# zyddnys/manga-image-translator

Hardware: AMD Instinct MI355X
Metric: pages/sec end-to-end (detect+OCR+inpaint), 2048x1456 (higher is better)
Workload: dtype f32

## Files before the change

manga_image_translator_amd/csrc/conv_gemm.hip:

```cpp
#include "conv_gemm_table.h"
#include <atomic>

using namespace mitcg;

#define G(name, fam, BM, BN, BK, ...) \
    extern template void mitcg::launch_##fam##_group<BM, BN, BK, __VA_ARGS__>(const mitcg::GroupArgs &, int, int, hipStream_t);
#include "conv_gemm_group_cfgs.inc"
#undef G

namespace {

int64_t max_a_offset(const MitConvGemm &p) {
    if (p.a_bs < 0 || p.a_ys < 0 || p.a_xs < 0) return -1;
    int tmax = 0;
    for (int t = 0; t < p.ntaps; ++t) {
        if (p.tap_off[t] < 0) return -1;
        if (p.tap_off[t] > tmax) tmax = p.tap_off[t];
    }
    return (int64_t)(p.NB - 1) * p.a_bs + (int64_t)(p.Hi - 1) * p.a_ys + (int64_t)(p.Wi - 1) * p.a_xs + p.Cin + tmax;
}
bool fast_eligible(const MitConvGemm &p, int BK) {
    if (p.Cin % BK || p.ntaps > FAST_MAX_TAPS) return false;
    const int64_t maxoff = max_a_offset(p);
    return maxoff >= 0 && maxoff < 0x7fffffffLL;
}

bool split_eligible(const MitConvGemm &p, int BK) {
    if (!p.w_split || (reinterpret_cast<uintptr_t>(p.w_split) & 15) || (p.ws_zs0 & 7)) return false;
    if (p.w_zs1 != 0 || (p.Kw & 7) || p.ntaps * p.Cin > p.Kw) return false;
    if ((int64_t)3 * (p.Kw >> 3) * p.ldw > 0x7fffffffLL) return false;
    return fast_eligible(p, BK);
}

bool buf_eligible(const MitConvGemm &p) {
    const int64_t maxoff = max_a_offset(p);
    return maxoff >= 0 && maxoff * 4 < 0x80000000LL && (int64_t)3 * (p.Kw >> 3) * p.ldw * 16 < 0x80000000LL;
}
int buf_form(const MitConvGemm &p, int c) { return buf_eligible(p) ? kCfgs[c].twin : c; }

bool gemv_eligible(const MitConvGemm &p, int lpr) {
    if (p.N > 4 || p.Z != 1 || p.Cin % (4 * lpr) || (int64_t)p.NB * p.Ho > 65535) return false;
    if ((int64_t)p.ntaps * p.Cin * (p.N == 1 ? 1 : 4) * 4 > 60 * 1024) return false;
    if (p.c.nsplit || p.pre.nsplit || p.post.nsplit || p.lut_rows) return false;
    return true;
}

std::atomic<int> g_gemm_mode{-1};
int gemm_mode_now() {
    int m = g_gemm_mode.load(std::memory_order_relaxed);
    if (m < 0) {
        const char *v = getenv("MIT_GEMM_SPLIT");
        m = (v && *v) ? atoi(v) : 6;
        if (m != 6 && m != 9) m = 0;
        g_gemm_mode.store(m, std::memory_order_relaxed);
    }
    return m;
}

std::atomic<long long> g_split_min{0};
int64_t split_min_now() { return g_split_min.load(std::memory_order_relaxed); }

struct TileSet {
    int n32;
    int narrow, wide;
    int small;
    int64_t small_max;
    int small_k32;
};
constexpr TileSet kGenericTiles = {CFG("128x32x16"), CFG("128x64x16"), CFG("128x128x16"), -1, 0, -1};
constexpr TileSet kFp32Tiles = {CFG("fast128x32x16w4c"), CFG("fast128x64x16w5c"), CFG("fast128x128x16w4c"), CFG("fast64x64x16w8c"), 1280, -1};
constexpr TileSet kP6Tiles = {CFG("split128x32x16p6o"), CFG("split128x64x16p6o"), CFG("split128x128x16p6o"), CFG("split64x64x16p6o"), 768, CFG("split64x64x32p6o")};
constexpr TileSet kP9Tiles = {CFG("split128x32x16p9m"), CFG("split128x64x16p9"), CFG("split128x128x16p9m"), CFG("split64x64x16p9m"), 768, CFG("split64x64x32p9m")};
constexpr TileSet kP1Tiles = {-1, CFG("split128x64x32p1o"), CFG("split128x128x32p1o"), CFG("split64x64x32p1o"), 768, -1};

int64_t tiles128(const MitConvGemm &p, int64_t M) { return ((M + 127) / 128) * ((p.N + 63) / 64); }

int ladder(const TileSet &s, const MitConvGemm &p, int64_t M, int exact = -1) {
    if (p.N <= 32 && s.n32 >= 0) return s.n32;
    const int rem = p.N % 128;
    int c = (p.N <= 64 || (rem != 0 && rem <= 64)) ? s.narrow : s.wide;
    if (exact >= 0) c = exact;
    if (s.small >= 0 && p.Z == 1 && tiles128(p, M) < s.small_max) {
        c = s.small;
        if (s.small_k32 >= 0 && ((M + 63) / 64) * ((p.N + 63) / 64) <= 512 && split_eligible(p, 32)) c = s.small_k32;
    }
    return c;
}

int exact_n_p6(const MitConvGemm &p) {
    if (p.Z != 1) return -1;
    const int K = p.ntaps * p.Cin;
    if ((p.N == 160 || p.N == 320) && K >= 512) return CFG("split128x160x16p6o");
    if (p.N > 64 && p.N <= 96 && K >= 256) return CFG("split128x96x16p6o");
    if (p.N == 192 && K >= 256) return CFG("split128x192x16p6o");
    return -1;
}

int pick_cfg(const MitConvGemm &p, int64_t M) {
    if (p.nprod == 1) {
        if (!split_eligible(p, 32)) return buf_form(p, CFG("split64x64x16p1o"));
        return buf_form(p, ladder(kP1Tiles, p, M, p.N % 192 == 0 ? CFG("split128x192x32p1o") : -1));
    }
    if (gemv_eligible(p, 16)) return p.N == 1 ? CFG("gemv16n1") : CFG("gemv16");
    if (gemv_eligible(p, 4)) return p.N == 1 ? CFG("gemv4n1") : CFG("gemv4");
    const int mode = gemm_mode_now();
    if ((mode == 6 || mode == 9) && p.w_split && split_eligible(p, 16) && tiles128(p, M) * p.Z >= split_min_now())
        return buf_form(p, mode == 6 ? ladder(kP6Tiles, p, M, exact_n_p6(p)) : ladder(kP9Tiles, p, M));
    if (!fast_eligible(p, 16)) return ladder(kGenericTiles, p, M);
    if (p.N > 32 && M > 128 && M <= 192 && p.Z >= 8) return CFG("fast192x64x16w4c");
    return ladder(kFp32Tiles, p, M);
}

struct ProbeRec {
    hipEvent_t start, stop;
    int cfg;
    double exec_flops, alg_flops;
    int M, N, K, ntaps, Z, act;
    double wino_bytes;
};
std::mutex g_probe_mu;
bool g_probe_on = false;
std::vector<ProbeRec> g_probe;
thread_local double g_next_alg_flops = -1.0;

}

extern "C" int mit_prof_enable(int on) {
    std::lock_guard<std::mutex> lk(g_probe_mu);
    for (auto &r : g_probe) {
        (void)hipEventDestroy(r.start);
        (void)hipEventDestroy(r.stop);
    }
    g_probe.clear();
    g_probe_on = on != 0;
    mit_probe_reset(on != 0);
    return 0;
}

extern "C" int mit_prof_tag_next(double alg_flops) {
    g_next_alg_flops = alg_flops;
    return 0;
}

extern "C" int mit_prof_dump(const char *path) {
    if (!path) return mit_set_error("mit_prof_dump: null path");
    std::lock_guard<std::mutex> lk(g_probe_mu);
    FILE *f = fopen(path, "w");
    if (!f) return mit_set_error("mit_prof_dump: cannot open %s", path);
    fprintf(f, "tile,M,N,K,taps,Z,act,ms,exec_flops,alg_flops,wino_bytes\n");
    for (auto &r : g_probe) {
        float ms = 0.f;
        if (hipEventSynchronize(r.stop) != hipSuccess || hipEventElapsedTime(&ms, r.start, r.stop) != hipSuccess) {
            fclose(f);
            return mit_set_error("mit_prof_dump: event query failed");
        }
        fprintf(f, "%s,%d,%d,%d,%d,%d,%d,%.6f,%.0f,%.0f,%.0f\n", kCfgs[r.cfg].name, r.M, r.N, r.K, r.ntaps, r.Z, r.act, ms, r.exec_flops,
                r.alg_flops, r.wino_bytes);
    }
    fclose(f);
    return 0;
}

extern "C" int mit_prof_read(MitProfStat *stats, int max_cfgs, int *n_cfgs) {
    if (!stats || !n_cfgs) return mit_set_error("mit_prof_read: null");
    std::lock_guard<std::mutex> lk(g_probe_mu);
    const int n = max_cfgs < kNumCfgs ? max_cfgs : kNumCfgs;
    for (int i = 0; i < n; ++i) {
        stats[i].launches = 0;
        stats[i].ms = stats[i].exec_flops = stats[i].alg_flops = 0.0;
    }
    for (auto &r : g_probe) {
        MIT_CHECK_HIP(hipEventSynchronize(r.stop));
        float ms = 0.f;
        MIT_CHECK_HIP(hipEventElapsedTime(&ms, r.start, r.stop));
        if (r.cfg < n) {
            stats[r.cfg].launches += 1;
            stats[r.cfg].ms += ms;
            stats[r.cfg].exec_flops += r.exec_flops;
            stats[r.cfg].alg_flops += r.alg_flops;
        }
    }
    *n_cfgs = n;
    return 0;
}

extern "C" const char *mit_conv_gemm_config_name(int cfg) {
    if (cfg < 0 || cfg >= kNumCfgs) return nullptr;
    return kCfgs[cfg].name;
}

extern "C" const char *mit_conv_gemm_config_kernel(int cfg) {
    if (cfg < 0 || cfg >= kNumCfgs) return nullptr;
    return kCfgs[cfg].kernel;
}

namespace {
bool map_vec_ok(const MitTensorMap &m, bool split_ok = false) {
    if (m.nsplit != 0 && !(split_ok && !(m.nsplit & 3) && !(m.nhi & 3))) return false;
    return !(reinterpret_cast<uintptr_t>(m.base) & 15) && !((m.zs1 | m.zs0 | m.bs | m.ys | m.xs) & 3);
}
bool vec_epilogue_ok(const MitConvGemm &p) {
    if ((p.N & 3) || !map_vec_ok(p.c, true)) return false;
    if (p.pre.base && !map_vec_ok(p.pre)) return false;
    if (p.post.base && !map_vec_ok(p.post)) return false;
    if (p.lut_rows && ((p.lut_ld & 3) || (reinterpret_cast<uintptr_t>(p.lut1) & 15) || (reinterpret_cast<uintptr_t>(p.lut2) & 15))) return false;
    return !(reinterpret_cast<uintptr_t>(p.scale) & 15) && !(reinterpret_cast<uintptr_t>(p.bias) & 15);
}

int64_t list_rows(const MitConvGemm &p) { return (int64_t)p.NB * ((p.Ho + 7) / 8) * ((p.Wo + 7) / 8) * 64; }
int64_t rows_of(const MitConvGemm &p) { return p.live_blocks ? list_rows(p) : (int64_t)p.NB * p.Ho * p.Wo; }

int validate(const MitConvGemm *d, MitConvGemm &p) {
    if (!d) return mit_set_error("mit_conv_gemm: null descriptor");
    p = *d;
    if (p.act & MIT_ACT_VEC_OK) return mit_set_error("mit_conv_gemm: reserved activation bits set");
    if (vec_epilogue_ok(p)) p.act |= MIT_ACT_VEC_OK;
    if (!p.a || !p.w || !p.c.base) return mit_set_error("mit_conv_gemm: null operand");
    if (p.Cin <= 0 || (p.Cin & 3)) return mit_set_error("mit_conv_gemm: Cin must be a positive multiple of 4 (got %d)", p.Cin);
    if ((p.ldw & 3) || (p.Nw & 3)) return mit_set_error("mit_conv_gemm: ldw/Nw must be multiples of 4 (ldw=%lld Nw=%d)", (long long)p.ldw, p.Nw);
    if (p.ntaps <= 0 || p.ntaps > MIT_MAX_TAPS) return mit_set_error("mit_conv_gemm: ntaps %d out of range", p.ntaps);
    if (p.NB <= 0 || p.Ho <= 0 || p.Wo <= 0 || p.N <= 0 || p.Z <= 0 || p.zdiv <= 0)
        return mit_set_error("mit_conv_gemm: empty problem");
    if ((reinterpret_cast<uintptr_t>(p.a) & 15) || (reinterpret_cast<uintptr_t>(p.w) & 15))
        return mit_set_error("mit_conv_gemm: operands must be 16-byte aligned");
    if ((p.a_xs & 3) || (p.a_ys & 3) || (p.a_bs & 3) || (p.a_zs0 & 3) || (p.a_zs1 & 3) || (p.w_zs0 & 3) || (p.w_zs1 & 3))
        return mit_set_error("mit_conv_gemm: strides must be multiples of 4 elements");
    for (int t = 0; t < p.ntaps; ++t)
        if (p.tap_off[t] & 3) return mit_set_error("mit_conv_gemm: tap_off must be multiples of 4");
    if (p.pad_mode == MIT_PAD_REFLECT) {
        for (int t = 0; t < p.ntaps; ++t) {
            int ady = p.tap_dy[t] < 0 ? -p.tap_dy[t] : p.tap_dy[t];
            int adx = p.tap_dx[t] < 0 ? -p.tap_dx[t] : p.tap_dx[t];
            if (ady >= p.Hi || adx >= p.Wi) return mit_set_error("mit_conv_gemm: reflect pad larger than input");
        }
    }
    if ((int64_t)p.NB * p.Ho * p.Wo > 0x7fffffffLL) return mit_set_error("mit_conv_gemm: M too large");
    if (p.lut_rows) {
        if (!p.lut1 || !p.lut2 || p.lut_ld < p.N) return mit_set_error("mit_conv_gemm: lut_rows needs lut1, lut2 and lut_ld >= N");
        if (p.Z != 1) return mit_set_error("mit_conv_gemm: the row-lookup epilogue is for Z == 1 launches");
        if (p.lut_ld > 0x7fff) return mit_set_error("mit_conv_gemm: lut_ld too large (row offsets are 16-bit row x lut_ld in 32 bits)");
    }
    if (p.live_blocks || p.live_start) {
        if (!p.live_blocks || !p.live_start) return mit_set_error("mit_conv_gemm: a live-block list needs live_blocks and live_start");
        if ((reinterpret_cast<uintptr_t>(p.live_blocks) | reinterpret_cast<uintptr_t>(p.live_start)) & 3) return mit_set_error("mit_conv_gemm: live_blocks / live_start must be 4-byte aligned");
        if (p.Z != 1) return mit_set_error("mit_conv_gemm: a live-block list is for Z == 1 launches");
        if (p.lut_rows) return mit_set_error("mit_conv_gemm: a live-block list together with lut_rows is not implemented");
        if (p.live_img0 < 0) return mit_set_error("mit_conv_gemm: live_img0 must be >= 0 (got %d)", p.live_img0);
        if (list_rows(p) > 0x7fffffffLL) return mit_set_error("mit_conv_gemm: M too large");
    } else if (p.live_img0 != 0) {
        return mit_set_error("mit_conv_gemm: live_img0 without a live-block list");
    }
    if (p.wino_m) {
        if (!p.live_blocks) return mit_set_error("mit_conv_gemm: wino_m needs the 8 x 8 block row order (live_blocks / live_start; list every block for a dense layer)");
        if (p.ntaps != 1 || p.sy != 1 || p.sx != 1) return mit_set_error("mit_conv_gemm: wino_m is for one tap with stride 1 (got %d taps, stride %d x %d)", p.ntaps, p.sy, p.sx);
        if (p.pre.base) return mit_set_error("mit_conv_gemm: wino_m together with a pre operand is not implemented");
        if (p.c.nsplit || (p.post.base && p.post.nsplit)) return mit_set_error("mit_conv_gemm: wino_m with a column-split map is not implemented");
        if ((p.N & 3) || p.wino_n != p.N) return mit_set_error("mit_conv_gemm: wino_m needs N %% 4 == 0 and wino_n == N (N=%d wino_n=%d)", p.N, p.wino_n);
        if (p.wino_th != (p.Ho + 3) / 4 || p.wino_tw != (p.Wo + 3) / 4)
            return mit_set_error("mit_conv_gemm: wino_th x wino_tw must be ceil(Ho / 4) x ceil(Wo / 4) (got %d x %d for %d x %d)", p.wino_th, p.wino_tw, p.Ho, p.Wo);
        if (p.wino_zs < (int64_t)p.NB * p.wino_th * p.wino_tw * p.wino_n) return mit_set_error("mit_conv_gemm: wino_zs is shorter than one slice of tiles (NB * wino_th * wino_tw * wino_n)");
        if (reinterpret_cast<uintptr_t>(p.wino_m) & 3) return mit_set_error("mit_conv_gemm: wino_m must be 4-byte aligned");
    }
    if (p.Z > 65535) return mit_set_error("mit_conv_gemm: Z too large");
    if (p.nprod != 0 && p.nprod != 1) return mit_set_error("mit_conv_gemm: nprod must be 0 (the GEMM mode) or 1 (one bf16 product) (got %d)", p.nprod);
    if (p.nprod == 1 && !p.w_split) return mit_set_error("mit_conv_gemm: nprod = 1 needs w_split (mit_gemm_split_pack): there is no fp32 fallback for a requested precision");
    return 0;
}

int images_per_run(const MitConvGemm &p) {
    if (p.Z != 1 || p.NB <= 1) return p.NB;
    MitConvGemm q = p;
    q.NB = 1;
    const bool want_buf = (gemm_mode_now() == 6 || p.nprod == 1) && p.w_split != nullptr && split_eligible(p, 16) && buf_eligible(q);
    auto run_ok = [&](const MitConvGemm &r) { return fast_eligible(r, 16) && (!want_buf || buf_eligible(r)); };
    if (p.Cin % 16 != 0 || p.ntaps > FAST_MAX_TAPS || p.a_bs <= 0 || run_ok(p) || !fast_eligible(q, 16)) return p.NB;
    int nb = p.NB;
    while (nb > 1) {
        q.NB = nb;
        if (run_ok(q)) break;
        nb = (nb + 1) / 2;
    }
    return nb;
}
MitConvGemm run_of(const MitConvGemm &p, int b0, int nb) {
    MitConvGemm r = p;
    r.NB = nb;
    r.a += (int64_t)b0 * p.a_bs;
    r.c.base += (int64_t)b0 * p.c.bs;
    if (p.pre.base) r.pre.base += (int64_t)b0 * p.pre.bs;
    if (p.post.base) r.post.base += (int64_t)b0 * p.post.bs;
    if (p.lut_rows) r.lut_rows += (int64_t)b0 * p.Ho * p.Wo;
    if (p.wino_m) r.wino_m += (int64_t)b0 * p.wino_th * p.wino_tw * p.wino_n;
    if (p.live_blocks) r.live_start += b0, r.live_img0 += b0;
    return r;
}

int plan_run(const MitConvGemm &p, int cfg, int *tile) {
    const int64_t M = rows_of(p);
    if (p.nprod == 1) {
        if (!split_eligible(p, 16))
            return mit_set_error("mit_conv_gemm: nprod = 1 needs the split tiles' preconditions (Cin %% 16 == 0, <= %d taps, 32-bit element offsets, 16-byte aligned w_split with w_zs1 == 0 and Kw %% 8 == 0): there is no fp32 fallback for a requested precision", FAST_MAX_TAPS);
        if (cfg >= 0 && cfg < kNumCfgs && kCfgs[cfg].nprod() != 1) return mit_set_error("mit_conv_gemm: nprod = 1 with tile %s, which is not a one-product tile", kCfgs[cfg].name);
    }
    if (cfg < 0) cfg = pick_cfg(p, M);
    if (cfg >= kNumCfgs) return mit_set_error("mit_conv_gemm: bad cfg %d", cfg);
    const CfgEntry &c = kCfgs[cfg];
    const bool fast = c.family == TileFamily::fast, split = c.family == TileFamily::split, gemv = c.family == TileFamily::gemv;
    if (p.lut_rows) {
        if (!fast && !split)
            return mit_set_error("mit_conv_gemm: the row-lookup epilogue (lut_rows) needs a fast or split tile (Cin %% 16 == 0, <= %d taps); this launch takes %s", FAST_MAX_TAPS, c.name);
        if (!(p.act & MIT_ACT_VEC_OK)) return mit_set_error("mit_conv_gemm: lut_rows needs the float4 epilogue (N %% 4 == 0, 16-byte aligned maps, tables and lut_ld %% 4 == 0)");
        if (p.post.base) return mit_set_error("mit_conv_gemm: lut_rows together with a post residual is not implemented");
        if ((p.act & 0xff) != MIT_ACT_NONE && (p.act & 0xff) != MIT_ACT_RELU) return mit_set_error("mit_conv_gemm: lut_rows is implemented for act none / relu");
    }
    if (p.live_blocks && !fast && !split)
        return mit_set_error("mit_conv_gemm: a live-block list needs a fast or split tile (Cin %% 16 == 0, <= %d taps, N > 4); this launch takes %s", FAST_MAX_TAPS, c.name);
    if (gemv && (!gemv_eligible(p, c.lanes_per_row()) || p.N > c.BN))
        return mit_set_error("mit_conv_gemm: cfg %s needs N <= %d, Z == 1, unsplit maps and Cin %% %d == 0", c.name, c.BN, 4 * c.lanes_per_row());
    if (split && !split_eligible(p, c.BK))
        return mit_set_error("mit_conv_gemm: cfg %s needs w_split (mit_gemm_split_pack, 16-byte aligned, w_zs1 == 0, Kw %% 8 == 0) and the fast tiles' preconditions", c.name);
    if (fast && !fast_eligible(p, c.BK))
        return mit_set_error("mit_conv_gemm: cfg %s needs Cin %% %d == 0, <= %d taps and 32-bit element offsets", c.name, c.BK, FAST_MAX_TAPS);
    if ((M + c.BM - 1) / c.BM * ((p.N + c.BN - 1) / c.BN) > 0x7fffffffLL) return mit_set_error("mit_conv_gemm: grid too large");
    *tile = cfg;
    return 0;
}

int launch_run(const MitConvGemm &p, int cfg, hipStream_t hs) {
    const CfgEntry &c = kCfgs[cfg];
    const int M = (int)rows_of(p);
    const int MT = (M + c.BM - 1) / c.BM;
    const int NT = (p.N + c.BN - 1) / c.BN;
    const int Ktot = p.ntaps * p.Cin;
    const int KT = (Ktot + c.BK - 1) / c.BK;
    const double tagged = g_next_alg_flops;
    g_next_alg_flops = -1.0;
    if (g_probe_on) {
        std::lock_guard<std::mutex> lk(g_probe_mu);
        ProbeRec r;
        MIT_CHECK_HIP(hipEventCreate(&r.start));
// ... 235 lines not shown
```

manga_image_translator_amd/csrc/conv_gemm_cfgs.inc:

```
X(0, "128x128x16", generic, 128, 128, 16, 2, 2)
X(0, "128x64x16", generic, 128, 64, 16, 2, 2)
X(0, "128x32x16", generic, 128, 32, 16, 4, 1)
X(1, "fast128x128x16w4c", fast, 128, 128, 16, 1, 4, 4, 4)
X(1, "fast128x64x16w5c", fast, 128, 64, 16, 2, 2, 5, 4)
X(1, "fast192x64x16w4c", fast, 192, 64, 16, 2, 2, 4, 4)
X(1, "fast64x64x16w8c", fast, 64, 64, 16, 2, 2, 8, 4)
X(1, "fast128x32x16w4c", fast, 128, 32, 16, 4, 1, 4, 4)
X(0, "gemv16", gemv, 8, 4, 4, 16)
X(0, "gemv4", gemv, 8, 4, 4, 4)
X(0, "gemv16n1", gemv, 8, 1, 4, 16)
X(0, "gemv4n1", gemv, 4, 1, 4, 4)
X(4, "split128x128x16p6o", split, 128, 128, 16, 2, 2, 3, 6, 385)
X(4, "split128x128x16p9m", split, 128, 128, 16, 2, 2, 3, 9, 129)
X(4, "split128x64x16p6o", split, 128, 64, 16, 2, 2, 3, 6, 385)
X(3, "split128x64x16p9", split, 128, 64, 16, 2, 2, 2, 9, 0)
X(3, "split64x64x16p6o", split, 64, 64, 16, 2, 2, 4, 6, 385)
X(3, "split64x64x16p9m", split, 64, 64, 16, 2, 2, 4, 9, 129)
X(3, "split64x64x32p6o", split, 64, 64, 32, 2, 2, 3, 6, 385)
X(3, "split64x64x32p9m", split, 64, 64, 32, 2, 2, 3, 9, 129)
X(3, "split128x32x16p6o", split, 128, 32, 16, 4, 1, 4, 6, 385)
X(3, "split128x32x16p9m", split, 128, 32, 16, 4, 1, 4, 9, 129)
X(3, "split128x160x16p6o", split, 128, 160, 16, 4, 1, 2, 6, 385)
X(3, "split128x96x16p6o", split, 128, 96, 16, 4, 1, 3, 6, 385)
X(3, "split128x192x16p6o", split, 128, 192, 16, 4, 1, 2, 6, 385)
X(2, "split128x128x16p6u", split, 128, 128, 16, 2, 2, 3, 6, 2433)
X(2, "split128x64x16p6u", split, 128, 64, 16, 2, 2, 3, 6, 2433)
X(2, "split64x64x16p6u", split, 64, 64, 16, 2, 2, 4, 6, 2433)
X(2, "split64x64x32p6u", split, 64, 64, 32, 2, 2, 3, 6, 2433)
X(5, "split128x32x16p6u", split, 128, 32, 16, 4, 1, 4, 6, 2433)
X(5, "split128x160x16p6u", split, 128, 160, 16, 4, 1, 2, 6, 2433)
X(5, "split128x96x16p6u", split, 128, 96, 16, 4, 1, 3, 6, 2433)
X(5, "split128x192x16p6u", split, 128, 192, 16, 4, 1, 2, 6, 2433)
X(3, "split128x128x16p6", split, 128, 128, 16, 2, 2, 2, 6, 0)
X(3, "split128x128x16p9", split, 128, 128, 16, 2, 2, 2, 9, 0)
X(3, "split128x128x16p3", split, 128, 128, 16, 2, 2, 2, 3, 0)
X(3, "split128x64x16p6", split, 128, 64, 16, 2, 2, 2, 6, 0)
X(6, "split128x128x32p1o", split, 128, 128, 32, 2, 2, 3, 1, 385)
X(6, "split128x128x32p1u", split, 128, 128, 32, 2, 2, 3, 1, 2433)
X(6, "split128x64x32p1o", split, 128, 64, 32, 2, 2, 3, 1, 385)
X(6, "split128x64x32p1u", split, 128, 64, 32, 2, 2, 3, 1, 2433)
X(6, "split128x192x32p1o", split, 128, 192, 32, 4, 1, 2, 1, 385)
X(6, "split128x192x32p1u", split, 128, 192, 32, 4, 1, 2, 1, 2433)
X(6, "split64x64x32p1o", split, 64, 64, 32, 2, 2, 4, 1, 385)
X(6, "split64x64x32p1u", split, 64, 64, 32, 2, 2, 4, 1, 2433)
X(6, "split64x64x16p1o", split, 64, 64, 16, 2, 2, 4, 1, 385)
X(6, "split64x64x16p1u", split, 64, 64, 16, 2, 2, 4, 1, 2433)
```

manga_image_translator_amd/csrc/conv_gemm_group_cfgs.inc:

```
G("128x128x16", generic, 128, 128, 16, 2, 2)
G("128x64x16", generic, 128, 64, 16, 2, 2)
G("fast128x128x16w4c", fast, 128, 128, 16, 1, 4, 4, 4)
G("fast128x64x16w5c", fast, 128, 64, 16, 2, 2, 5, 4)
G("fast64x64x16w8c", fast, 64, 64, 16, 2, 2, 8, 4)
G("split128x64x16p6u", split, 128, 64, 16, 2, 2, 3, 6, 2433)
G("split64x64x16p6u", split, 64, 64, 16, 2, 2, 4, 6, 2433)
G("split64x64x32p6u", split, 64, 64, 32, 2, 2, 3, 6, 2433)
G("split128x160x16p6u", split, 128, 160, 16, 4, 1, 2, 6, 2433)
G("split128x96x16p6u", split, 128, 96, 16, 4, 1, 3, 6, 2433)
```

manga_image_translator_amd/csrc/conv_gemm_split.h:

```cpp
#pragma once
#include "bf16_split.h"

namespace mitcg {


template <int BK>
__device__ __forceinline__ constexpr int split_swz(int kh) { return kh * (64 / BK); }

template <int BM, int BN, int BK, int WAVES_M, int WAVES_N, int NPROD, int VAR, class P>
__device__ __forceinline__ void conv_gemm_split_body(const P &p, const int M, const int MT, const int NT, const int KT, const int cur_tile) {
    constexpr int WM = BM / WAVES_M;
    constexpr int WN = BN / WAVES_N;
    constexpr int TM = WM / 32;
    constexpr int TN = WN / 32;
    static_assert(WAVES_M * WAVES_N == 4 && TM >= 1 && TN >= 1, "wave tile");
    static_assert(BK == 16 || BK == 32, "K-tile of one or two bf16 MFMA steps");
    static_assert(NPROD == 1 || NPROD == 3 || NPROD == 6 || NPROD == 9, "plane pairs");
    constexpr int NPL = NPROD == 1 ? 1 : 3;
    constexpr int KH = BK / 8;
    constexpr int KS = BK / 16;
    constexpr int KQ = BK / 4;
    constexpr int A_ITERS = BM * KQ / 256;
    constexpr int A_MSTEP = 256 / KQ;
    static_assert(A_ITERS >= 1 && (BM * KQ) % 256 == 0, "A tile must fill the workgroup");
    constexpr bool PIPE = (VAR & 1) != 0;
    static_assert(PIPE == ((VAR & 128) != 0), "the pipelined schedule is the stepped one (VAR 1 + 128)");
    constexpr bool ORD = (VAR & 256) != 0;
    constexpr bool BUF = (VAR & 2048) != 0;
    static_assert((VAR & ~(1 | 128 | 256 | 2048)) == 0, "VAR bits");
    constexpr int SA = BM, SB = BN;
    constexpr int A_TILE = NPL * KH * SA, B_TILE = NPL * KH * SB;
    constexpr int B_CPP = KH * BN;
    constexpr int B_CELLS = NPL * B_CPP;
    constexpr int B_ITERS = (B_CELLS + 255) / 256;

    extern __shared__ __attribute__((aligned(16))) float smem[];
    u32x4 *As = reinterpret_cast<u32x4 *>(smem);
    u32x4 *Bs = As + 2 * A_TILE;
    int *rowtab = reinterpret_cast<int *>(Bs + 2 * B_TILE);

    const int tid = threadIdx.x;
    const int lane = tid & 63;
    const int wave = __builtin_amdgcn_readfirstlane(tid >> 6);
    const int li = lane & 31;
    const int lh = lane >> 5;

    int m0 = 0, n0 = 0;
    const int z = blockIdx.y;
    const int z1 = z / p.zdiv, z0 = z - z1 * p.zdiv;
    const int HoWo = p.Ho * p.Wo;

    const float *__restrict__ a_base = p.a + z1 * p.a_zs1 + z0 * p.a_zs0;
    const u32x4 *__restrict__ ws = reinterpret_cast<const u32x4 *>(p.w_split + z0 * p.ws_zs0);
    const int K8 = p.Kw >> 3;
    const int ldn = (int)p.ldw;

    const int aq = tid % KQ;
    const int am = tid / KQ;
    const float *__restrict__ a_thr = a_base + aq * 4;
    const __amdgpu_buffer_rsrc_t ra = __builtin_amdgcn_make_buffer_rsrc(const_cast<float *>(a_base), 0, 0x80000000u, 0x00020000);
    const __amdgpu_buffer_rsrc_t rw = __builtin_amdgcn_make_buffer_rsrc(const_cast<u32x4 *>(ws), 0, 0x80000000u, 0x00020000);
    const int aq16 = aq * 16;
    constexpr bool B_UNI = B_CPP == 256;
    constexpr int B_IDX = B_UNI ? 1 : B_ITERS;
    int b_src[B_IDX], b_dst[B_IDX];
    bool b_ok[B_IDX];
    auto bsrc = [&](const int i) { return B_UNI ? b_src[0] + i * K8 * ldn : b_src[B_UNI ? 0 : i]; };
    auto bdst = [&](const int i) { return B_UNI ? b_dst[0] + i * KH * SB : b_dst[B_UNI ? 0 : i]; };
    auto bok = [&](const int i) { return b_ok[B_UNI ? 0 : i]; };
    int ld_tap = 0, ld_ci0 = 0, ld_k8 = 0;
    auto setup_tile = [&](const int t) {
        const int mt = t / NT, nt = t - mt * NT;
        m0 = mt * BM;
        n0 = nt * BN;
        for (int idx = tid; idx < p.ntaps * BM; idx += 256) {
            const int tp = idx / BM, r = idx - tp * BM;
            const int m = m0 + r;
            int off = -1;
            int nb, oy, ox;
            if (decode_row(p, m, M, HoWo, nb, oy, ox)) {
                int iy = oy * p.sy + p.tap_dy[tp];
                int ix = ox * p.sx + p.tap_dx[tp];
                bool ok = true;
                if (p.pad_mode == MIT_PAD_REFLECT) {
                    iy = iy < 0 ? -iy : (iy >= p.Hi ? 2 * p.Hi - 2 - iy : iy);
                    ix = ix < 0 ? -ix : (ix >= p.Wi ? 2 * p.Wi - 2 - ix : ix);
                } else {
                    ok = iy >= 0 && iy < p.Hi && ix >= 0 && ix < p.Wi;
                }
                if (ok) off = (int)((int64_t)nb * p.a_bs + (int64_t)iy * p.a_ys + (int64_t)ix * p.a_xs + p.tap_off[tp]);
            }
            rowtab[idx] = BUF ? (off < 0 ? (int)0x80000000u : off * 4) : off;
        }
#pragma unroll
        for (int i = 0; i < B_IDX; ++i) {
            const int c = tid + i * 256;
            const int pl = c / B_CPP, rem = c - pl * B_CPP;
            const int kh = rem / BN, n = rem - kh * BN;
            b_ok[i] = c < B_CELLS && (n0 + n) < ldn;
            b_src[i] = (pl * K8 + kh) * ldn + n0 + n;
            b_dst[i] = (pl * KH + kh) * SB + n;
        }
        ld_tap = ld_ci0 = ld_k8 = 0;
    };
    setup_tile(cur_tile);

    f32x4 a_reg[A_ITERS];
    u32x4 b_reg[B_ITERS];
    int a_off[A_ITERS];

    __syncthreads();

    auto load_tile = [&]() {
        const int *rt = rowtab + ld_tap * BM + am;
#pragma unroll
        for (int i = 0; i < A_ITERS; ++i) a_off[i] = rt[i * A_MSTEP];
        const float *ak = a_thr + ld_ci0;
#pragma unroll
        for (int i = 0; i < A_ITERS; ++i) {
            if (BUF) a_reg[i] = __builtin_bit_cast(f32x4, __builtin_amdgcn_raw_buffer_load_b128(ra, a_off[i] + aq16, ld_ci0 * 4, 0));
            else a_reg[i] = *reinterpret_cast<const f32x4 *>(ak + (a_off[i] < 0 ? 0 : a_off[i]));
        }
        const u32x4 *wk = ws + (int64_t)ld_k8 * ldn;
#pragma unroll
        for (int i = 0; i < B_ITERS; ++i) {
            if (BUF) b_reg[i] = __builtin_amdgcn_raw_buffer_load_b128(rw, bok(i) ? bsrc(i) * 16 : -1, ld_k8 * ldn * 16, 0);
            else b_reg[i] = wk[bok(i) ? bsrc(i) : 0];
        }
        ld_k8 += KH;
        ld_ci0 += BK;
        const bool wrap = ld_ci0 >= p.Cin;
        ld_ci0 = wrap ? 0 : ld_ci0;
        ld_tap += wrap ? 1 : 0;
    };
    auto store_tile = [&](int buf) {
        u32x2 *as2 = reinterpret_cast<u32x2 *>(As + buf * A_TILE);
        const int kh = aq >> 1, half = aq & 1;
#pragma unroll
        for (int i = 0; i < A_ITERS; ++i) {
            const int ml = (am + i * A_MSTEP) ^ split_swz<BK>(kh);
            u32x2 h, m, l;
            const f32x4 zero = {0.f, 0.f, 0.f, 0.f};
            const f32x4 v = !BUF && a_off[i] < 0 ? zero : a_reg[i];
            if (NPL == 1) {
                as2[(kh * SA + ml) * 2 + half] = u32x2{pack_bf16(v.x, v.y), pack_bf16(v.z, v.w)};
                continue;
            }
            split3(v, h, m, l);
            as2[((0 * KH + kh) * SA + ml) * 2 + half] = h;
            as2[((1 * KH + kh) * SA + ml) * 2 + half] = m;
            as2[((2 * KH + kh) * SA + ml) * 2 + half] = l;
        }
        u32x4 *bs = Bs + buf * B_TILE;
#pragma unroll
        for (int i = 0; i < B_ITERS; ++i)
            if ((i + 1) * 256 <= B_CELLS || tid + i * 256 < B_CELLS) bs[bdst(i)] = b_reg[i];
    };

    f32x16 acc[TM][TN];

    const int wm0 = (wave / WAVES_N) * WM;
    const int wn0 = (wave % WAVES_N) * WN;

    constexpr int STAGE_WRITE_STEPS = NPL * A_ITERS + B_ITERS, STAGE_STEPS = STAGE_WRITE_STEPS + 1 + A_ITERS + B_ITERS;
    auto stage_step = [&](const int st, const int buf, const bool with_loads) {
        if (ORD && st == NPL * (A_ITERS - 1) + 1 && with_loads) {
            const int *rt = rowtab + ld_tap * BM + am;
#pragma unroll
            for (int i = 0; i < A_ITERS; ++i) a_off[i] = rt[i * A_MSTEP];
        }
        if (st < NPL * A_ITERS) {
            const int i = st / NPL, ph = st % NPL;
            const int kh = aq >> 1, half = aq & 1;
            static_assert((A_MSTEP & (A_MSTEP - 1)) == 0 && (BK / 4) * (32 / (BK / 4)) <= A_MSTEP || A_ITERS == 1, "row swizzle must stay inside a chunk's rows");
            const int ml = ((am ^ split_swz<BK>(kh)) + i * A_MSTEP);
            f32x4 &r = a_reg[i];
            if (ph == 0 && !BUF) {
                const unsigned int keep = ~(unsigned int)(a_off[i] >> 31);
                r.x = __uint_as_float(__float_as_uint(r.x) & keep);
                r.y = __uint_as_float(__float_as_uint(r.y) & keep);
                r.z = __uint_as_float(__float_as_uint(r.z) & keep);
                r.w = __uint_as_float(__float_as_uint(r.w) & keep);
            }
            const u32x2 pk = {pack_bf16(r.x, r.y), pack_bf16(r.z, r.w)};
            reinterpret_cast<u32x2 *>(As + buf * A_TILE)[((ph * KH + kh) * SA + ml) * 2 + half] = pk;
            if (ph < NPL - 1) {
                r.x = r.x - bf16_lo(pk.x);
                r.y = r.y - bf16_hi(pk.x);
                r.z = r.z - bf16_lo(pk.y);
                r.w = r.w - bf16_hi(pk.y);
            }
        } else if (st < STAGE_WRITE_STEPS) {
            const int j = st - NPL * A_ITERS;
            if ((j + 1) * 256 <= B_CELLS || tid + j * 256 < B_CELLS) (Bs + buf * B_TILE)[bdst(j)] = b_reg[j];
        } else if (st == STAGE_WRITE_STEPS) {
            if (!ORD) {
                const int *rt = rowtab + ld_tap * BM + am;
#pragma unroll
                for (int i = 0; i < A_ITERS; ++i) a_off[i] = rt[i * A_MSTEP];
            }
        } else if (st <= STAGE_WRITE_STEPS + A_ITERS) {
            const int i = st - STAGE_WRITE_STEPS - 1;
            if (BUF) a_reg[i] = __builtin_bit_cast(f32x4, __builtin_amdgcn_raw_buffer_load_b128(ra, a_off[i] + aq16, ld_ci0 * 4, 0));
            else a_reg[i] = *reinterpret_cast<const f32x4 *>(a_thr + ld_ci0 + (a_off[i] < 0 ? 0 : a_off[i]));
        } else if (st < STAGE_STEPS) {
            const int j = st - STAGE_WRITE_STEPS - 1 - A_ITERS;
            if (BUF) b_reg[j] = __builtin_amdgcn_raw_buffer_load_b128(rw, bok(j) ? bsrc(j) * 16 : -1, ld_k8 * ldn * 16, 0);
            else b_reg[j] = (ws + (int64_t)ld_k8 * ldn)[bok(j) ? bsrc(j) : 0];
            if (st == STAGE_STEPS - 1) {
                ld_k8 += KH;
                ld_ci0 += BK;
                const bool wrap = ld_ci0 >= p.Cin;
                ld_ci0 = wrap ? 0 : ld_ci0;
                ld_tap += wrap ? 1 : 0;
            }
        }
    };

    bf16x8 af[KS][NPL][TM], bf[KS][NPL][TN];
    auto tile = [&](const int kt, auto do_store, auto do_load) {
        constexpr bool DO_STORE = decltype(do_store)::value, DO_LOAD = decltype(do_load)::value;
        const int cur = kt & 1;
        if (!PIPE && DO_STORE) load_tile();
        const u32x4 *as = As + cur * A_TILE;
        const u32x4 *bs = Bs + cur * B_TILE + lh * SB + wn0 + li;
#pragma unroll
        for (int ks = 0; ks < KS; ++ks)
#pragma unroll
            for (int o = 0; o < NPL; ++o) {
                const int pa = ORD && NPL == 3 ? (o == 0 ? 0 : 3 - o) : o;
                const int pb = ORD && NPL == 3 ? (o == 0 ? 2 : o - 1) : o;
#pragma unroll
                for (int mi = 0; mi < TM; ++mi)
                    af[ks][pa][mi] = __builtin_bit_cast(bf16x8, as[(pa * KH + 2 * ks + lh) * SA + ((wm0 + mi * 32 + li) ^ split_swz<BK>(2 * ks + lh))]);
#pragma unroll
                for (int ni = 0; ni < TN; ++ni) bf[ks][pb][ni] = __builtin_bit_cast(bf16x8, bs[(pb * KH + 2 * ks) * SB + ni * 32]);
            }
        if (PIPE) {
            constexpr int NM = KS * NPROD * TM * TN;
            constexpr int NSTEP = DO_STORE ? (DO_LOAD ? STAGE_STEPS : STAGE_WRITE_STEPS) : 0;
#pragma unroll
            for (int i = 0; i < NM; ++i) {
                const int ni = i % TN, mi = (i / TN) % TM, pr = 9 - NPROD + (i / (TN * TM)) % NPROD, ks = i / (TN * TM * NPROD);
                acc[mi][ni] = __builtin_amdgcn_mfma_f32_32x32x16_bf16(af[ks][kSplitPA[pr]][mi], bf[ks][kSplitPB[pr]][ni], acc[mi][ni], 0, 0, 0);
                if (i >= 1 && i - 1 < NSTEP) stage_step(i - 1, cur ^ 1, DO_LOAD);
                __builtin_amdgcn_sched_barrier(0);
            }
#pragma unroll
            for (int st = NM - 1; st < NSTEP; ++st) stage_step(st, cur ^ 1, DO_LOAD);
        } else {
#pragma unroll
            for (int ks = 0; ks < KS; ++ks)
#pragma unroll
                for (int pr = 9 - NPROD; pr < 9; ++pr)
#pragma unroll
                    for (int mi = 0; mi < TM; ++mi)
#pragma unroll
                        for (int ni = 0; ni < TN; ++ni)
                            acc[mi][ni] = __builtin_amdgcn_mfma_f32_32x32x16_bf16(af[ks][kSplitPA[pr]][mi], bf[ks][kSplitPB[pr]][ni], acc[mi][ni], 0, 0, 0);
            if (DO_STORE) store_tile(cur ^ 1);
        }
        __syncthreads();
    };
    const std::integral_constant<bool, true> yes;
    const std::integral_constant<bool, false> no;

    constexpr int EPI_FLOATS = (BM * (int)sizeof(RowOff) + 15) / 16 * 4 + 4 * 32 * EPI_PITCH + BM * (int)sizeof(LutOff) / 4;
    constexpr int STAGE_FLOATS = (2 * A_TILE + 2 * B_TILE) * 4;
    constexpr int SMEM_F = STAGE_FLOATS > EPI_FLOATS ? STAGE_FLOATS : EPI_FLOATS;

    load_tile();
#pragma unroll
    for (int mi = 0; mi < TM; ++mi)
#pragma unroll
        for (int ni = 0; ni < TN; ++ni)
#pragma unroll
            for (int r = 0; r < 16; ++r) acc[mi][ni][r] = 0.f;
    store_tile(0);
    if (PIPE && KT > 1) load_tile();
    __syncthreads();
    {
        int kt = 0;
        if (PIPE) {
            for (; kt + 2 < KT; ++kt) tile(kt, yes, yes);
            if (kt + 1 < KT) tile(kt++, yes, no);
        } else {
            for (; kt + 1 < KT; ++kt) tile(kt, yes, no);
        }
        tile(kt, no, no);
    }
    const int tid_e = wave * 64 + (int)__builtin_amdgcn_mbcnt_hi(~0u, __builtin_amdgcn_mbcnt_lo(~0u, 0u));
    epilogue<BM, TM, TN, SMEM_F, 256, true>(p, acc, smem, M, m0, n0, wm0, wn0, z1, z0, HoWo, tid_e);
}
template <int BM, int BN, int BK, int WAVES_M, int WAVES_N, int MINW, int NPROD, int VAR>
__global__ __launch_bounds__(256, MINW) void conv_gemm_split_kernel(const MitConvGemm p, const int M, const int MT, const int NT,
                                                                  const int KT) {
    const int nwg = live_workgroups<BM>(p, MT, NT);
    if ((int)blockIdx.x >= nwg) return;
    conv_gemm_split_body<BM, BN, BK, WAVES_M, WAVES_N, NPROD, VAR>(p, M, MT, NT, KT, xcd_tile((int)blockIdx.x, nwg));
}
template <int BM, int BN, int BK, int WAVES_M, int WAVES_N, int MINW, int NPROD, int VAR>
__global__ __launch_bounds__(256, MINW) void conv_gemm_split_kernel_group(const GroupArgs g, const int NT, const int KT) {
    MIT_GROUP_PROLOGUE(BM);
    conv_gemm_split_body<BM, BN, BK, WAVES_M, WAVES_N, NPROD, VAR>(v, M, MT, NT, KT, tile);
}


static __global__ __launch_bounds__(256) void gemm_split_pack_kernel(const float *__restrict__ w, const int64_t w_zs, const int K8, const int ldw,
                                                              uint16_t *__restrict__ out, const int64_t total) {
    const int64_t idx = (int64_t)blockIdx.x * 256 + threadIdx.x;
    if (idx >= total) return;
    const int n = (int)(idx % ldw);
    const int64_t t = idx / ldw;
    const int k8 = (int)(t % K8);
    const int64_t z = t / K8;
    const float *src = w + z * w_zs + (int64_t)k8 * 8 * ldw + n;
    unsigned int h[4], m[4], l[4];
#pragma unroll
    for (int j = 0; j < 4; ++j) {
        const float x0 = src[(int64_t)(2 * j) * ldw], x1 = src[(int64_t)(2 * j + 1) * ldw];
        h[j] = pack_bf16(x0, x1);
        const float r0 = x0 - bf16_lo(h[j]), r1 = x1 - bf16_hi(h[j]);
        m[j] = pack_bf16(r0, r1);
        l[j] = pack_bf16(r0 - bf16_lo(m[j]), r1 - bf16_hi(m[j]));
    }
    const int64_t plane = (int64_t)K8 * ldw;
    u32x4 *o = reinterpret_cast<u32x4 *>(out) + z * 3 * plane + (int64_t)k8 * ldw + n;
    o[0] = u32x4{h[0], h[1], h[2], h[3]};
    o[plane] = u32x4{m[0], m[1], m[2], m[3]};
    o[2 * plane] = u32x4{l[0], l[1], l[2], l[3]};
}

template <int BM, int BN, int BK, int WAVES_M, int WAVES_N, int MINW, int NPROD, int VAR>
void launch_split(const MitConvGemm &p, int M, int MT, int NT, int KT, hipStream_t s) {
    constexpr int KH = BK / 8;
    constexpr int SA = BM, SB = BN;
    constexpr int NPL = NPROD == 1 ? 1 : 3;
    size_t staging = (size_t)(2 * NPL * KH * SA + 2 * NPL * KH * SB) * 16 + (size_t)p.ntaps * BM * sizeof(int);
    size_t rows = ((size_t)BM * sizeof(RowOff) + 15) / 16 * 16 + (size_t)4 * 32 * EPI_PITCH * sizeof(float) + (size_t)BM * sizeof(LutOff);
    size_t smem = staging > rows ? staging : rows;
    auto kern = conv_gemm_split_kernel<BM, BN, BK, WAVES_M, WAVES_N, MINW, NPROD, VAR>;
    static DynSmemOptIn optin;
    optin.ensure(reinterpret_cast<const void *>(kern), smem);
    dim3 grid(MT * NT, p.Z, 1);
    hipLaunchKernelGGL(kern, grid, dim3(256), smem, s, p, M, MT, NT, KT);
}
template <int BM, int BN, int BK, int WAVES_M, int WAVES_N, int MINW, int NPROD, int VAR>
void launch_split_group(const GroupArgs &g, int NT, int KT, hipStream_t s) {
    constexpr int KH = BK / 8;
    constexpr int SA = BM, SB = BN;
    constexpr int NPL = NPROD == 1 ? 1 : 3;
    size_t staging = (size_t)(2 * NPL * KH * SA + 2 * NPL * KH * SB) * 16 + (size_t)g.p.ntaps * BM * sizeof(int);
    size_t rows = ((size_t)BM * sizeof(RowOff) + 15) / 16 * 16 + (size_t)4 * 32 * EPI_PITCH * sizeof(float) + (size_t)BM * sizeof(LutOff);
    size_t smem = staging > rows ? staging : rows;
    auto kern = conv_gemm_split_kernel_group<BM, BN, BK, WAVES_M, WAVES_N, MINW, NPROD, VAR>;
    static DynSmemOptIn optin;
    optin.ensure(reinterpret_cast<const void *>(kern), smem);
    hipLaunchKernelGGL(kern, dim3(g.tile0[g.n]), dim3(256), smem, s, g, NT, KT);
}

}
```

manga_image_translator_amd/csrc/conv_gemm_table.h:

```cpp
#pragma once
#include "conv_gemm_kernels.h"
#include <string_view>

namespace mitcg {
enum class TileFamily { generic, fast, gemv, split };
struct CfgEntry {
    const char *name;
    TileFamily family;
    int BM, BN, BK;
    int args[5];
    void (*launch)(const MitConvGemm &, int M, int MT, int NT, int KT, hipStream_t);
    const char *kernel;
    int twin;
    constexpr int nprod() const { return family == TileFamily::split ? args[3] : 0; }
    constexpr bool buf() const { return family == TileFamily::split && (args[4] & 2048) != 0; }
    constexpr int lanes_per_row() const { return family == TileFamily::gemv ? args[0] : 0; }
};
}

#define X(g, name, fam, BM, BN, BK, ...) \
    extern template void mitcg::launch_##fam<BM, BN, BK, __VA_ARGS__>(const MitConvGemm &, int, int, int, int, hipStream_t);
#include "conv_gemm_cfgs.inc"
#undef X

namespace mitcg {
namespace {

#define KNAME_generic "conv_gemm_kernel"
#define KNAME_fast "conv_gemm_fast_kernel"
#define KNAME_gemv "conv_gemv_kernel"
#define KNAME_split "conv_gemm_split_kernel"
constexpr CfgEntry kCfgRows[] = {
#define X(g, name, fam, BM, BN, BK, ...) \
    {name, TileFamily::fam, BM, BN, BK, {__VA_ARGS__}, launch_##fam<BM, BN, BK, __VA_ARGS__>, KNAME_##fam "<" #BM ", " #BN ", " #BK ", " #__VA_ARGS__ ">", 0},
#include "conv_gemm_cfgs.inc"
#undef X
};
constexpr int kNumCfgs = sizeof(kCfgRows) / sizeof(kCfgRows[0]);
static_assert(kNumCfgs < 64, "the probe's callers size their arrays for 64 tiles");

constexpr bool is_buf_twin(const CfgEntry &a, const CfgEntry &b) {
    return a.family == TileFamily::split && b.family == a.family && !a.buf() && a.BM == b.BM && a.BN == b.BN && a.BK == b.BK && a.args[0] == b.args[0] &&
           a.args[1] == b.args[1] && a.args[2] == b.args[2] && a.args[3] == b.args[3] && b.args[4] == a.args[4] + 2048;
}
struct CfgTable {
    CfgEntry e[kNumCfgs];
};
constexpr CfgTable kCfgTable = [] {
    CfgTable t{};
    for (int i = 0; i < kNumCfgs; ++i) {
        t.e[i] = kCfgRows[i];
        t.e[i].twin = i;
        for (int j = 0; j < kNumCfgs; ++j)
            if (is_buf_twin(kCfgRows[i], kCfgRows[j])) t.e[i].twin = j;
    }
    return t;
}();
constexpr const CfgEntry (&kCfgs)[kNumCfgs] = kCfgTable.e;

constexpr int find_cfg(std::string_view name) {
    for (int i = 0; i < kNumCfgs; ++i)
        if (name == kCfgRows[i].name) return i;
    return -1;
}
#define CFG(name) ([] { constexpr int i = find_cfg(name); static_assert(i >= 0, "no tile " name " in conv_gemm_cfgs.inc"); return i; }())
static_assert(CFG("128x128x16") == 0 && kCfgs[CFG("split64x64x32p1o")].twin == CFG("split64x64x32p1u") && kCfgs[CFG("split128x64x16p9")].twin == CFG("split128x64x16p9"), "table order, buffer-load twins");

}
}
```

Measured before the change: 48.15.

## Add gather-free plain path for 1x1 stride-1 split GEMM tiles

Adds a PLAIN variant bit to the buffer-load split conv-GEMM kernel. For single-tap, unit-stride, contiguous inputs it computes A-row offsets directly in registers instead of building a shared-memory row table, and skips the setup barrier. The weight load is also issued before the row setup so it overlaps. The host chooses the plain instantiation at launch only when eligibility checks pass, otherwise it falls back, which doubles the template instantiations and compile time.

```diff
diff --git a/manga_image_translator_amd/csrc/conv_gemm.hip b/manga_image_translator_amd/csrc/conv_gemm.hip
--- a/manga_image_translator_amd/csrc/conv_gemm.hip
+++ b/manga_image_translator_amd/csrc/conv_gemm.hip
@@ -36,6 +36,21 @@
     const int64_t maxoff = max_a_offset(p);
     return maxoff >= 0 && maxoff * 4 < 0x80000000LL && (int64_t)3 * (p.Kw >> 3) * p.ldw * 16 < 0x80000000LL;
 }
+}
+static bool plain_dims(const MitConvGemm &p, int NB, int Hi, int Wi, int Ho, int Wo, int64_t a_bs, int64_t a_ys) {
+    if (p.ntaps != 1 || p.sy != 1 || p.sx != 1 || p.tap_dy[0] != 0 || p.tap_dx[0] != 0 || p.live_blocks) return false;
+    if (Ho > Hi || Wo > Wi || p.a_xs <= 0) return false;
+    if (Ho > 1 && a_ys != (int64_t)Wo * p.a_xs) return false;
+    if (NB > 1 && a_bs != (int64_t)Ho * Wo * p.a_xs) return false;
+    return true;
+}
+bool mitcg::plain_eligible(const MitConvGemm &p) { return buf_eligible(p) && plain_dims(p, p.NB, p.Hi, p.Wi, p.Ho, p.Wo, p.a_bs, p.a_ys); }
+bool mitcg::plain_eligible_member(const MitConvGemm &b, const MitConvGemmMember &m) {
+    MitConvGemm d = b;
+    d.a = m.a, d.a_bs = m.a_bs, d.a_ys = m.a_ys, d.NB = m.NB, d.Hi = m.Hi, d.Wi = m.Wi, d.Ho = m.Ho, d.Wo = m.Wo;
+    return buf_eligible(d) && plain_dims(d, d.NB, d.Hi, d.Wi, d.Ho, d.Wo, d.a_bs, d.a_ys);
+}
+namespace {
 int buf_form(const MitConvGemm &p, int c) { return buf_eligible(p) ? kCfgs[c].twin : c; }
 
 bool gemv_eligible(const MitConvGemm &p, int lpr) {
diff --git a/manga_image_translator_amd/csrc/conv_gemm_cfgs.inc b/manga_image_translator_amd/csrc/conv_gemm_cfgs.inc
--- a/manga_image_translator_amd/csrc/conv_gemm_cfgs.inc
+++ b/manga_image_translator_amd/csrc/conv_gemm_cfgs.inc
@@ -23,14 +23,14 @@
 X(3, "split128x160x16p6o", split, 128, 160, 16, 4, 1, 2, 6, 385)
 X(3, "split128x96x16p6o", split, 128, 96, 16, 4, 1, 3, 6, 385)
 X(3, "split128x192x16p6o", split, 128, 192, 16, 4, 1, 2, 6, 385)
-X(2, "split128x128x16p6u", split, 128, 128, 16, 2, 2, 3, 6, 2433)
-X(2, "split128x64x16p6u", split, 128, 64, 16, 2, 2, 3, 6, 2433)
-X(2, "split64x64x16p6u", split, 64, 64, 16, 2, 2, 4, 6, 2433)
-X(2, "split64x64x32p6u", split, 64, 64, 32, 2, 2, 3, 6, 2433)
-X(5, "split128x32x16p6u", split, 128, 32, 16, 4, 1, 4, 6, 2433)
-X(5, "split128x160x16p6u", split, 128, 160, 16, 4, 1, 2, 6, 2433)
-X(5, "split128x96x16p6u", split, 128, 96, 16, 4, 1, 3, 6, 2433)
-X(5, "split128x192x16p6u", split, 128, 192, 16, 4, 1, 2, 6, 2433)
+X(2,"split128x128x16p6u", split, 128, 128, 16, 2, 2, 3, 6, 6529)
+X(2, "split128x64x16p6u", split, 128, 64, 16, 2, 2, 3, 6, 6529)
+X(2, "split64x64x16p6u", split, 64, 64, 16, 2, 2, 4, 6, 6529)
+X(2, "split64x64x32p6u", split, 64, 64, 32, 2, 2, 3, 6, 6529)
+X(5, "split128x32x16p6u", split, 128, 32, 16, 4, 1, 4, 6, 6529)
+X(5, "split128x160x16p6u", split, 128, 160, 16, 4, 1, 2, 6, 6529)
+X(5, "split128x96x16p6u", split, 128, 96, 16, 4, 1, 3, 6, 6529)
+X(5, "split128x192x16p6u", split, 128, 192, 16, 4, 1, 2, 6, 6529)
 X(3, "split128x128x16p6", split, 128, 128, 16, 2, 2, 2, 6, 0)
 X(3, "split128x128x16p9", split, 128, 128, 16, 2, 2, 2, 9, 0)
 X(3, "split128x128x16p3", split, 128, 128, 16, 2, 2, 2, 3, 0)
diff --git a/manga_image_translator_amd/csrc/conv_gemm_group_cfgs.inc b/manga_image_translator_amd/csrc/conv_gemm_group_cfgs.inc
--- a/manga_image_translator_amd/csrc/conv_gemm_group_cfgs.inc
+++ b/manga_image_translator_amd/csrc/conv_gemm_group_cfgs.inc
@@ -3,8 +3,8 @@
 G("fast128x128x16w4c", fast, 128, 128, 16, 1, 4, 4, 4)
 G("fast128x64x16w5c", fast, 128, 64, 16, 2, 2, 5, 4)
 G("fast64x64x16w8c", fast, 64, 64, 16, 2, 2, 8, 4)
-G("split128x64x16p6u", split, 128, 64, 16, 2, 2, 3, 6, 2433)
-G("split64x64x16p6u", split, 64, 64, 16, 2, 2, 4, 6, 2433)
-G("split64x64x32p6u", split, 64, 64, 32, 2, 2, 3, 6, 2433)
-G("split128x160x16p6u", split, 128, 160, 16, 4, 1, 2, 6, 2433)
-G("split128x96x16p6u", split, 128, 96, 16, 4, 1, 3, 6, 2433)
+G("split128x64x16p6u", split, 128, 64, 16, 2, 2, 3, 6, 6529)
+G("split64x64x16p6u", split, 64, 64, 16, 2, 2, 4, 6, 6529)
+G("split64x64x32p6u", split, 64, 64, 32, 2, 2, 3, 6, 6529)
+G("split128x160x16p6u", split, 128, 160, 16, 4, 1, 2, 6, 6529)
+G("split128x96x16p6u", split, 128, 96, 16, 4, 1, 3, 6, 6529)
diff --git a/manga_image_translator_amd/csrc/conv_gemm_split.h b/manga_image_translator_amd/csrc/conv_gemm_split.h
--- a/manga_image_translator_amd/csrc/conv_gemm_split.h
+++ b/manga_image_translator_amd/csrc/conv_gemm_split.h
@@ -27,7 +27,9 @@
     static_assert(PIPE == ((VAR & 128) != 0), "the pipelined schedule is the stepped one (VAR 1 + 128)");
     constexpr bool ORD = (VAR & 256) != 0;
     constexpr bool BUF = (VAR & 2048) != 0;
-    static_assert((VAR & ~(1 | 128 | 256 | 2048)) == 0, "VAR bits");
+    constexpr bool PLAIN = (VAR & 4096) != 0;
+    static_assert(!PLAIN || BUF, "the gather-free path marks dead rows through the buffer descriptor's range check");
+    static_assert((VAR & ~(1 | 128 | 256 | 2048 | 4096)) == 0, "VAR bits");
     constexpr int SA = BM, SB = BN;
     constexpr int A_TILE = NPL * KH * SA, B_TILE = NPL * KH * SB;
     constexpr int B_CPP = KH * BN;
@@ -69,10 +71,34 @@
     auto bdst = [&](const int i) { return B_UNI ? b_dst[0] + i * KH * SB : b_dst[B_UNI ? 0 : i]; };
     auto bok = [&](const int i) { return b_ok[B_UNI ? 0 : i]; };
     int ld_tap = 0, ld_ci0 = 0, ld_k8 = 0;
-    auto setup_tile = [&](const int t) {
+    f32x4 a_reg[A_ITERS];
+    u32x4 b_reg[B_ITERS];
+    int a_off[A_ITERS];
+    auto setup_w = [&](const int t) {
         const int mt = t / NT, nt = t - mt * NT;
         m0 = mt * BM;
         n0 = nt * BN;
+#pragma unroll
+        for (int i = 0; i < B_IDX; ++i) {
+            const int c = tid + i * 256;
+            const int pl = c / B_CPP, rem = c - pl * B_CPP;
+            const int kh = rem / BN, n = rem - kh * BN;
+            b_ok[i] = c < B_CELLS && (n0 + n) < ldn;
+            b_src[i] = (pl * K8 + kh) * ldn + n0 + n;
+            b_dst[i] = (pl * KH + kh) * SB + n;
+        }
+        ld_tap = ld_ci0 = ld_k8 = 0;
+    };
+    auto setup_rows = [&]() {
+        if (PLAIN) {
+            const int xs4 = (int)p.a_xs * 4, t4 = p.tap_off[0] * 4;
+#pragma unroll
+            for (int i = 0; i < A_ITERS; ++i) {
+                const int m = m0 + am + i * A_MSTEP;
+                a_off[i] = m < M ? m * xs4 + t4 : (int)0x80000000u;
+            }
+            return;
+        }
         for (int idx = tid; idx < p.ntaps * BM; idx += 256) {
             const int tp = idx / BM, r = idx - tp * BM;
             const int m = m0 + r;
@@ -92,46 +118,40 @@
             }
             rowtab[idx] = BUF ? (off < 0 ? (int)0x80000000u : off * 4) : off;
         }
-#pragma unroll
-        for (int i = 0; i < B_IDX; ++i) {
-            const int c = tid + i * 256;
-            const int pl = c / B_CPP, rem = c - pl * B_CPP;
-            const int kh = rem / BN, n = rem - kh * BN;
-            b_ok[i] = c < B_CELLS && (n0 + n) < ldn;
-            b_src[i] = (pl * K8 + kh) * ldn + n0 + n;
-            b_dst[i] = (pl * KH + kh) * SB + n;
-        }
-        ld_tap = ld_ci0 = ld_k8 = 0;
-    };
-    setup_tile(cur_tile);
-
-    f32x4 a_reg[A_ITERS];
-    u32x4 b_reg[B_ITERS];
-    int a_off[A_ITERS];
-
-    __syncthreads();
-
-    auto load_tile = [&]() {
-        const int *rt = rowtab + ld_tap * BM + am;
-#pragma unroll
-        for (int i = 0; i < A_ITERS; ++i) a_off[i] = rt[i * A_MSTEP];
+    };
+
+    auto load_a = [&]() {
+        if (!PLAIN) {
+            const int *rt = rowtab + ld_tap * BM + am;
+#pragma unroll
+            for (int i = 0; i < A_ITERS; ++i) a_off[i] = rt[i * A_MSTEP];
+        }
         const float *ak = a_thr + ld_ci0;
 #pragma unroll
         for (int i = 0; i < A_ITERS; ++i) {
             if (BUF) a_reg[i] = __builtin_bit_cast(f32x4, __builtin_amdgcn_raw_buffer_load_b128(ra, a_off[i] + aq16, ld_ci0 * 4, 0));
             else a_reg[i] = *reinterpret_cast<const f32x4 *>(ak + (a_off[i] < 0 ? 0 : a_off[i]));
         }
+    };
+    auto load_w = [&]() {
         const u32x4 *wk = ws + (int64_t)ld_k8 * ldn;
 #pragma unroll
         for (int i = 0; i < B_ITERS; ++i) {
             if (BUF) b_reg[i] = __builtin_amdgcn_raw_buffer_load_b128(rw, bok(i) ? bsrc(i) * 16 : -1, ld_k8 * ldn * 16, 0);
             else b_reg[i] = wk[bok(i) ? bsrc(i) : 0];
         }
+    };
+    auto load_next = [&]() {
         ld_k8 += KH;
         ld_ci0 += BK;
         const bool wrap = ld_ci0 >= p.Cin;
         ld_ci0 = wrap ? 0 : ld_ci0;
         ld_tap += wrap ? 1 : 0;
+    };
+    auto load_tile = [&]() {
+        load_a();
+        load_w();
+        load_next();
     };
     auto store_tile = [&](int buf) {
         u32x2 *as2 = reinterpret_cast<u32x2 *>(As + buf * A_TILE);
@@ -164,7 +184,7 @@
 
     constexpr int STAGE_WRITE_STEPS = NPL * A_ITERS + B_ITERS, STAGE_STEPS = STAGE_WRITE_STEPS + 1 + A_ITERS + B_ITERS;
     auto stage_step = [&](const int st, const int buf, const bool with_loads) {
-        if (ORD && st == NPL * (A_ITERS - 1) + 1 && with_loads) {
+        if (!PLAIN && ORD && st == NPL * (A_ITERS - 1) + 1 && with_loads) {
             const int *rt = rowtab + ld_tap * BM + am;
 #pragma unroll
             for (int i = 0; i < A_ITERS; ++i) a_off[i] = rt[i * A_MSTEP];
@@ -194,7 +214,7 @@
             const int j = st - NPL * A_ITERS;
             if ((j + 1) * 256 <= B_CELLS || tid + j * 256 < B_CELLS) (Bs + buf * B_TILE)[bdst(j)] = b_reg[j];
         } else if (st == STAGE_WRITE_STEPS) {
-            if (!ORD) {
+            if (!ORD && !PLAIN) {
                 const int *rt = rowtab + ld_tap * BM + am;
 #pragma unroll
                 for (int i = 0; i < A_ITERS; ++i) a_off[i] = rt[i * A_MSTEP];
@@ -269,7 +289,12 @@
     constexpr int STAGE_FLOATS = (2 * A_TILE + 2 * B_TILE) * 4;
     constexpr int SMEM_F = STAGE_FLOATS > EPI_FLOATS ? STAGE_FLOATS : EPI_FLOATS;
 
-    load_tile();
+    setup_w(cur_tile);
+    load_w();
+    setup_rows();
+    if (!PLAIN) __syncthreads();
+    load_a();
+    load_next();
 #pragma unroll
     for (int mi = 0; mi < TM; ++mi)
 #pragma unroll
@@ -331,14 +356,22 @@
     o[2 * plane] = u32x4{l[0], l[1], l[2], l[3]};
 }
 
-template <int BM, int BN, int BK, int WAVES_M, int WAVES_N, int MINW, int NPROD, int VAR>
-void launch_split(const MitConvGemm &p, int M, int MT, int NT, int KT, hipStream_t s) {
+bool plain_eligible(const MitConvGemm &p);
+bool plain_eligible_member(const MitConvGemm &base, const MitConvGemmMember &m);
+constexpr int SPLIT_PLAIN = 4096;
+
+template <int BM, int BN, int BK, int NPROD>
+size_t split_smem(const int ntaps) {
     constexpr int KH = BK / 8;
     constexpr int SA = BM, SB = BN;
     constexpr int NPL = NPROD == 1 ? 1 : 3;
-    size_t staging = (size_t)(2 * NPL * KH * SA + 2 * NPL * KH * SB) * 16 + (size_t)p.ntaps * BM * sizeof(int);
+    size_t staging = (size_t)(2 * NPL * KH * SA + 2 * NPL * KH * SB) * 16 + (size_t)ntaps * BM * sizeof(int);
     size_t rows = ((size_t)BM * sizeof(RowOff) + 15) / 16 * 16 + (size_t)4 * 32 * EPI_PITCH * sizeof(float) + (size_t)BM * sizeof(LutOff);
-    size_t smem = staging > rows ? staging : rows;
+    return staging > rows ? staging : rows;
+}
+template <int BM, int BN, int BK, int WAVES_M, int WAVES_N, int MINW, int NPROD, int VAR>
+void launch_split_kernel(const MitConvGemm &p, int M, int MT, int NT, int KT, hipStream_t s) {
+    const size_t smem = split_smem<BM, BN, BK, NPROD>(p.ntaps);
     auto kern = conv_gemm_split_kernel<BM, BN, BK, WAVES_M, WAVES_N, MINW, NPROD, VAR>;
     static DynSmemOptIn optin;
     optin.ensure(reinterpret_cast<const void *>(kern), smem);
@@ -346,17 +379,28 @@
     hipLaunchKernelGGL(kern, grid, dim3(256), smem, s, p, M, MT, NT, KT);
 }
 template <int BM, int BN, int BK, int WAVES_M, int WAVES_N, int MINW, int NPROD, int VAR>
-void launch_split_group(const GroupArgs &g, int NT, int KT, hipStream_t s) {
-    constexpr int KH = BK / 8;
-    constexpr int SA = BM, SB = BN;
-    constexpr int NPL = NPROD == 1 ? 1 : 3;
-    size_t staging = (size_t)(2 * NPL * KH * SA + 2 * NPL * KH * SB) * 16 + (size_t)g.p.ntaps * BM * sizeof(int);
-    size_t rows = ((size_t)BM * sizeof(RowOff) + 15) / 16 * 16 + (size_t)4 * 32 * EPI_PITCH * sizeof(float) + (size_t)BM * sizeof(LutOff);
-    size_t smem = staging > rows ? staging : rows;
+void launch_split(const MitConvGemm &p, int M, int MT, int NT, int KT, hipStream_t s) {
+    if constexpr ((VAR & SPLIT_PLAIN) != 0) {
+        if (plain_eligible(p)) return launch_split_kernel<BM, BN, BK, WAVES_M, WAVES_N, MINW, NPROD, VAR>(p, M, MT, NT, KT, s);
+    }
+    launch_split_kernel<BM, BN, BK, WAVES_M, WAVES_N, MINW, NPROD, VAR & ~SPLIT_PLAIN>(p, M, MT, NT, KT, s);
+}
+template <int BM, int BN, int BK, int WAVES_M, int WAVES_N, int MINW, int NPROD, int VAR>
+void launch_split_group_kernel(const GroupArgs &g, int NT, int KT, hipStream_t s) {
+    const size_t smem = split_smem<BM, BN, BK, NPROD>(g.p.ntaps);
     auto kern = conv_gemm_split_kernel_group<BM, BN, BK, WAVES_M, WAVES_N, MINW, NPROD, VAR>;
     static DynSmemOptIn optin;
     optin.ensure(reinterpret_cast<const void *>(kern), smem);
     hipLaunchKernelGGL(kern, dim3(g.tile0[g.n]), dim3(256), smem, s, g, NT, KT);
 }
-
-}
+template <int BM, int BN, int BK, int WAVES_M, int WAVES_N, int MINW, int NPROD, int VAR>
+void launch_split_group(const GroupArgs &g, int NT, int KT, hipStream_t s) {
+    if constexpr ((VAR & SPLIT_PLAIN) != 0) {
+        bool plain = true;
+        for (int i = 0; i < g.n; ++i) plain = plain && plain_eligible_member(g.p, g.m[i]);
+        if (plain) return launch_split_group_kernel<BM, BN, BK, WAVES_M, WAVES_N, MINW, NPROD, VAR>(g, NT, KT, s);
+    }
+    launch_split_group_kernel<BM, BN, BK, WAVES_M, WAVES_N, MINW, NPROD, VAR & ~SPLIT_PLAIN>(g, NT, KT, s);
+}
+
+}
diff --git a/manga_image_translator_amd/csrc/conv_gemm_table.h b/manga_image_translator_amd/csrc/conv_gemm_table.h
--- a/manga_image_translator_amd/csrc/conv_gemm_table.h
+++ b/manga_image_translator_amd/csrc/conv_gemm_table.h
@@ -41,7 +41,7 @@
 
 constexpr bool is_buf_twin(const CfgEntry &a, const CfgEntry &b) {
     return a.family == TileFamily::split && b.family == a.family && !a.buf() && a.BM == b.BM && a.BN == b.BN && a.BK == b.BK && a.args[0] == b.args[0] &&
-           a.args[1] == b.args[1] && a.args[2] == b.args[2] && a.args[3] == b.args[3] && b.args[4] == a.args[4] + 2048;
+           a.args[1] == b.args[1] && a.args[2] == b.args[2] && a.args[3] == b.args[3] && (b.args[4] & ~4096) == a.args[4] + 2048;
 }
 struct CfgTable {
     CfgEntry e[kNumCfgs];
```

Result: no change. 48.55 (median of 6 runs) (+0.8%).
